# sedaprotocol/bn254

Hardware: AMD Instinct MI355X
Metric: BN254 pairings/sec (batch verify) (higher is better)
Workload: dtype u32

## Files before the change

### bn254_amd/csrc/bn254_hip.hip

```cpp
#include <hip/hip_runtime.h>
#include <thread>

#include <cstdio>
#include <cstdlib>
#include <cstring>
#include <new>

#include "../../include/bn254_hip.h"
#include "bn254_hash.h"
#include "bn254_io.h"
#include "bn254_pairing.h"

using namespace bn254;

#include "bn254_ws.h"
#include "bn254_lane.h"
#include "bn254_host.h"

KERNEL_SMALL void k_decode_g1(const uint8_t* pts, size_t n, uint32_t flags, Ws ws, int px, int inf_plane, int accumulate) {
  size_t i = (size_t)blockIdx.x * BN_WAVE + threadIdx.x;
  if (i >= n) return;
  G1Affine p;
  uint8_t st = decode_g1(p, pts + 64 * i, flags);
  if (st != ST_OK) g1_set_generator(p);
  ws_store_g1(ws, px, inf_plane, i, p);
  uint8_t prev = accumulate ? ws_byte(ws, BY_ST_DECODE, i) : (uint8_t)ST_OK;
  ws_byte(ws, BY_ST_DECODE, i) = prev != ST_OK ? prev : st;
}
KERNEL void k_decode_g2(const uint8_t* pts, size_t n, uint32_t flags, Ws ws, int accumulate) {
  size_t i = (size_t)blockIdx.x * BN_WAVE + threadIdx.x;
// ... 11 lines not shown
}

__device__ __forceinline__ bool msg_span(const uint64_t* off, size_t i, uint64_t msgs_len, uint64_t& lo, uint64_t& len) {
  lo = off[i];
  const uint64_t hi = off[i + 1];
  const bool ok = lo <= hi && hi <= msgs_len;
  len = ok ? hi - lo : 0;
  if (!ok) lo = 0;
  return ok;
}
KERNEL_SMALL void k_hash_init(size_t n, Ws ws) {
  size_t i = (size_t)blockIdx.x * BN_WAVE + threadIdx.x;
  if (i < n) { ws.h_best[i] = HASH_NONE; ws.h_next[i] = 0; }
  if (i <= HASH_MAX_ROUNDS) ws.h_cnt[i] = (i == 0) ? (uint32_t)n : 0u;
}
KERNEL_SMALL void k_hash_round(const uint8_t* msgs, const uint64_t* off, uint64_t msgs_len, Ws ws, int round, uint32_t width, uint32_t max_ctr) {
  const uint32_t n_act = ws.h_cnt[round];
  if (n_act == 0) return;
  const uint32_t* list = round == 0 ? nullptr : ws.h_list + (size_t)(round & 1) * ws.stride;
  const size_t total = (size_t)n_act * width;
  for (size_t w = (size_t)blockIdx.x * BN_WAVE + threadIdx.x; w < total; w += (size_t)gridDim.x * BN_WAVE) {
    uint32_t slot = (uint32_t)(w % n_act), j = (uint32_t)(w / n_act);
    uint32_t i = list ? list[slot] : slot;
    uint32_t ctr = (uint32_t)ws.h_next[i] + j;
    if (ctr >= max_ctr) continue;
    uint64_t lo, len;
    msg_span(off, i, msgs_len, lo, len);
    const uint8_t* msg = msgs + lo;
    HashState hs;
    hash_state_init(hs, msg, len);
    if (hash_try_filter(hs, msg, len, ctr)) atomicMin(&ws.h_best[i], ctr);
  }
}
KERNEL_SMALL void k_hash_resolve(Ws ws, int round, uint32_t width, uint32_t max_ctr, uint32_t mark) {
  const uint32_t n_act = ws.h_cnt[round];
  if (n_act == 0) return;
  const uint32_t* list = round == 0 ? nullptr : ws.h_list + (size_t)(round & 1) * ws.stride;
  uint32_t* list_out = ws.h_list + (size_t)((round + 1) & 1) * ws.stride;
  const size_t span = (size_t)gridDim.x * BN_WAVE;
  for (size_t base = (size_t)blockIdx.x * BN_WAVE; base < n_act; base += span) {
    const size_t slot = base + threadIdx.x;
    bool survivor = false;
    uint32_t i = 0;
    if (slot < n_act) {
      i = list ? list[slot] : (uint32_t)slot;
      if (ws.h_best[i] == HASH_NONE) {
        const uint32_t next = (uint32_t)ws.h_next[i] + width;
// ... 111 lines not shown
  ws_byte(ws, BY_ST_HASH, i) = ok ? (uint8_t)ST_OK : !span_ok ? (uint8_t)ST_INVALID_LENGTH : (uint8_t)ST_HASH_TO_POINT;
  if (tries_out) tries_out[i] = ok ? (uint8_t)(best + 1) : !span_ok ? (uint8_t)0 : (uint8_t)max_ctr;
}
KERNEL_SMALL void k_hash_finish(const uint8_t* msgs, const uint64_t* off, uint64_t msgs_len, size_t n, Ws ws, uint32_t max_ctr, int px, int inf_plane,
                                uint8_t* tries_out) {
  size_t i = (size_t)blockIdx.x * BN_WAVE + threadIdx.x;
  if (i >= n) return;
  hash_finish_item(msgs, off, msgs_len, i, ws, max_ctr, px, inf_plane, tries_out);
}
__device__ __noinline__ bool hash_try_msg(G1Affine& out, const uint8_t* msg, uint64_t len, uint32_t ctr) {
  HashState hs;
  hash_state_init(hs, msg, len);
  return hash_try(out, hs, msg, len, ctr);
}
KERNEL_SMALL void k_hash_finish_tail(const uint8_t* msgs, const uint64_t* off, uint64_t msgs_len, size_t n, Ws ws, uint32_t max_ctr, int px, int inf_plane,
                                     uint8_t* tries_out, unsigned nblk_finish, uint32_t chunk) {
  if (blockIdx.x < nblk_finish) {
    const size_t i = (size_t)blockIdx.x * BN_WAVE + threadIdx.x;
    if (i < n) hash_finish_item(msgs, off, msgs_len, i, ws, max_ctr, px, inf_plane, tries_out);
    return;
  }
  const uint32_t n_tail = ws.h_cnt[1];
  const uint32_t* list = ws.h_list + ws.stride;
  const uint32_t per_wave = BN_WAVE / chunk, sub = threadIdx.x / chunk, j = threadIdx.x % chunk;
  const size_t span = (size_t)(gridDim.x - nblk_finish) * per_wave;
  for (size_t base = (size_t)(blockIdx.x - nblk_finish) * per_wave; base < n_tail; base += span) {
    const size_t slot = base + sub;
    const bool live = slot < n_tail;
    uint32_t i = 0, first = 0;
    uint64_t lo = 0, len = 0;
    bool span_ok = true;
    if (live) { i = list[slot]; first = ws.h_next[i]; span_ok = msg_span(off, i, msgs_len, lo, len); }
    const uint8_t* msg = msgs + lo;
    bool open = live && span_ok;
    for (uint32_t k = 0;; k += chunk) {
      const uint32_t ctr = first + k + j;
      bool ok = false;
      G1Affine p;
// ... 323 lines not shown
  return 0;
}

int launch_decode_g2(bn254_ctx* c, hipStream_t s, const uint8_t* d_pts, size_t n, uint32_t flags, int accumulate) {
  if (c->pair_lanes && (flags & FLAG_G2_SUBGROUP_CHECK)) {
    if (route_lane_machine_helpers(c, n)) {
      k_decode_g2<<<grid_for(n), BN_WAVE, 0, s>>>(d_pts, n, flags & ~(uint32_t)FLAG_G2_SUBGROUP_CHECK, c->ws, accumulate);
      return bn254_lm_g2_subgroup(n, c->ws, s);
    }
    return bn254_pair_decode_g2(d_pts, n, flags, c->ws, accumulate, s);
  }
  k_decode_g2<<<grid_for(n), BN_WAVE, 0, s>>>(d_pts, n, flags, c->ws, accumulate);
  return 0;
}

static uint32_t hash_wide_width(size_t n) {
  double survivors = (double)n * 0.5274 * 0.5274 * 0.5274 * 0.5274;
  uint32_t w = 4;
  for (; w < 8 && (double)n / BN_WAVE + survivors * HASH_TAIL_CHUNK_DEFAULT / BN_WAVE > (double)HASH_WIDE_WAVES; ++w) survivors *= 0.5274;
  return w;
}
int launch_hash_rounds(bn254_ctx* c, hipStream_t s, const uint8_t* d_msgs, const uint64_t* d_off, size_t n, int px, int inf_plane,
                              uint8_t* d_tries, int mark_finish) {
  const uint32_t max_ctr = c->hash_max_tries ? (uint32_t)c->hash_max_tries : 255u;
  const uint64_t msgs_len = c->msgs_len_call;
  k_hash_init<<<grid_for(n > HASH_MAX_ROUNDS + 1 ? n : HASH_MAX_ROUNDS + 1), BN_WAVE, 0, s>>>(n, c->ws);
  if (n <= HASH_DIRECT_MAX_N && c->hash_direct_width > 0) {
    const uint32_t width = (uint32_t)c->hash_direct_width;
    k_hash_direct<<<grid_for(n * width), BN_WAVE, 0, s>>>(d_msgs, d_off, msgs_len, n, c->ws, width, max_ctr, px, inf_plane, d_tries);
    if (max_ctr > width)
      k_hash_round<<<grid_for(64 * (max_ctr - width)), BN_WAVE, 0, s>>>(d_msgs, d_off, msgs_len, c->ws, 1, max_ctr - width, max_ctr);
    if (mark_finish >= 0 && c->profiling) HIP_TRY(hipEventRecord(c->ev[mark_finish], s));
    k_hash_finish<<<grid_for(n), BN_WAVE, 0, s>>>(d_msgs, d_off, msgs_len, n, c->ws, max_ctr, px, inf_plane, d_tries);
    HIP_TRY(hipGetLastError());
    return 0;
  }
  if (n > HASH_DIRECT_MAX_N && (c->hash_schedule == 2 || (c->hash_schedule == 0 && n <= HASH_WIDE_MAX_N))) {
    uint32_t w0 = c->hash_wide_width ? (uint32_t)c->hash_wide_width : hash_wide_width(n);
    if (w0 > max_ctr) w0 = max_ctr;
    size_t lanes = n * w0;
    if (lanes > HASH_MAX_GRID_LANES) lanes = HASH_MAX_GRID_LANES;
    k_hash_round<<<grid_for(lanes), BN_WAVE, 0, s>>>(d_msgs, d_off, msgs_len, c->ws, 0, w0, max_ctr);
    if (n > HASH_RESOLVE_TILES_MIN) {
      size_t tiles = (n + HASH_RESOLVE_WG - 1) / HASH_RESOLVE_WG;
      if (tiles > 16384) tiles = 16384;
      k_hash_resolve_tiles<<<(unsigned)tiles, HASH_RESOLVE_WG, 0, s>>>(c->ws, 0, w0, max_ctr, HASH_TAIL);
    } else {
      k_hash_resolve<<<grid_for(n), BN_WAVE, 0, s>>>(c->ws, 0, w0, max_ctr, HASH_TAIL);
    }
    double pf = 1.0;
    for (uint32_t t = 0; t < w0 && pf > 1e-12; ++t) pf *= 0.5274;
    double bound = (double)n * pf * 1.25 + 256.0;
    if (bound > (double)n) bound = (double)n;
    const uint32_t chunk = (uint32_t)c->hash_tail_chunk;
    size_t tail_blocks = ((size_t)bound * chunk + BN_WAVE - 1) / BN_WAVE;
    if (tail_blocks > HASH_TAIL_MAX_BLOCKS) tail_blocks = HASH_TAIL_MAX_BLOCKS;
    if (mark_finish >= 0 && c->profiling) HIP_TRY(hipEventRecord(c->ev[mark_finish], s));
    const unsigned nblk = grid_for(n);
    k_hash_finish_tail<<<nblk + (unsigned)tail_blocks, BN_WAVE, 0, s>>>(d_msgs, d_off, msgs_len, n, c->ws, max_ctr, px, inf_plane, d_tries, nblk, chunk);
    HIP_TRY(hipGetLastError());
    return 0;
  }
  double expect = (double)n;
  uint32_t consumed = 0;
  for (int round = 0; round < HASH_MAX_ROUNDS && consumed < max_ctr; ++round) {
    bool last = round == HASH_MAX_ROUNDS - 1;
    double lanes_per_msg = (double)HASH_TARGET_LANES / (expect < 1.0 ? 1.0 : expect);
    uint32_t width = lanes_per_msg < 2.0 ? 1u : (uint32_t)lanes_per_msg;
    if (width > max_ctr - consumed || last) width = max_ctr - consumed;
    double bound = expect * 1.25 + 256.0;
    if (bound > (double)n) bound = (double)n;
    size_t lanes = (size_t)(bound * width);
    if (lanes > HASH_MAX_GRID_LANES) lanes = HASH_MAX_GRID_LANES;
    k_hash_round<<<grid_for(lanes), BN_WAVE, 0, s>>>(d_msgs, d_off, msgs_len, c->ws, round, width, max_ctr);
    if ((size_t)bound > HASH_RESOLVE_TILES_MIN) {
      size_t tiles = ((size_t)bound + HASH_RESOLVE_WG - 1) / HASH_RESOLVE_WG;
      if (tiles > 16384) tiles = 16384;
      k_hash_resolve_tiles<<<(unsigned)tiles, HASH_RESOLVE_WG, 0, s>>>(c->ws, round, width, max_ctr, HASH_NONE);
    } else {
      k_hash_resolve<<<grid_for((size_t)bound), BN_WAVE, 0, s>>>(c->ws, round, width, max_ctr, HASH_NONE);
    }
    consumed += width;
    double pf = 1.0;
    for (uint32_t t = 0; t < width && pf > 1e-12; ++t) pf *= 0.5274;
    expect *= pf;
  }
  if (mark_finish >= 0 && c->profiling) HIP_TRY(hipEventRecord(c->ev[mark_finish], s));
  k_hash_finish<<<grid_for(n), BN_WAVE, 0, s>>>(d_msgs, d_off, msgs_len, n, c->ws, max_ctr, px, inf_plane, d_tries);
  HIP_TRY(hipGetLastError());
  return 0;
}

int launch_decode_g1(bn254_ctx* c, hipStream_t s, const uint8_t* d_pts, size_t n, uint32_t flags, int px, int inf_plane, int accumulate) {
  k_decode_g1<<<grid_for(n), BN_WAVE, 0, s>>>(d_pts, n, flags, c->ws, px, inf_plane, accumulate);
  return 0;
}
int launch_miller_var_lane(bn254_ctx* c, hipStream_t s, size_t n) {
  k_miller_var<<<grid_for(n), BN_WAVE, 0, s>>>(n, c->ws);
  return 0;
}
int launch_miller_verify_lane(bn254_ctx* c, hipStream_t s, size_t n, const uint32_t* map, const uint32_t* count) {
// ... 29 lines not shown
  c->agg_rand_min_pairs = AGG_RAND_MIN_PAIRS_DEFAULT;
  c->agg_rand_group_pairs = AGG_RAND_GROUP_PAIRS_DEFAULT;
  c->bmr_min_tuples = BITMAP_RAND_MIN_TUPLES_DEFAULT;
  c->bmr_group_tuples = BITMAP_RAND_GROUP_TUPLES_DEFAULT;
  c->bmr_max_keys = BITMAP_RAND_MAX_KEYS_DEFAULT;
  c->collect_wave_min = COLLECT_WAVE_MIN_SHARES_DEFAULT;
  c->collect_rand_min_shares = COLLECT_RAND_MIN_SHARES_DEFAULT;
  c->collect_rand_min_per_key = COLLECT_RAND_MIN_PER_KEY_DEFAULT;
  c->collect_opt_min_shares = COLLECT_OPT_MIN_SHARES_DEFAULT;
  c->collect_opt_min_tuple_shares = COLLECT_OPT_MIN_TUPLE_SHARES_DEFAULT;
  c->merge_wave_min = MERGE_WAVE_MIN_PARTS_DEFAULT;
  c->merge_opt_min_parts = MERGE_OPT_MIN_PARTS_DEFAULT;
  c->trio_max_batch = TRIO_MAX_BATCH_DEFAULT;
  c->hash_direct_width = HASH_DIRECT_WIDTH_DEFAULT;
  c->hash_tail_chunk = HASH_TAIL_CHUNK_DEFAULT;
  c->trio_wave_roles = TRIO_WAVE_ROLES_DEFAULT;
  c->agg_subset_min_tuples = AGG_SUBSET_MIN_TUPLES_DEFAULT;
  c->agg_sort_by_msg = 1;
  c->agg_t4_route = 0;
  c->agg_wide_min_tuples = AGG_WIDE_MIN_TUPLES_DEFAULT;
  c->pinned_staging = PINNED_STAGING_DEFAULT;
  c->fits_w8 = bn254_quad_fits_device(1); c->fits_quad = bn254_quad_fits_device(0); c->fits_trio = bn254_trio_fits_device();
  if (c->trio_wave_roles == 2 && !c->fits_w8) c->trio_wave_roles = 1;
  if (c->trio_wave_roles == 1 && !c->fits_quad) c->trio_wave_roles = 0;
  if (!c->fits_trio) c->trio_max_batch = 0;
  c->nonet_max_batch = bn254_nonet_fits_device() ? NONET_MAX_BATCH_DEFAULT : 0;
  c->lm_max_batch = bn254_lm_fits_device() ? LM_MAX_BATCH_DEFAULT : 0;
  c->nonet_wide = 1;
  c->g2_fixed_base = 1;
  c->key_dedup = 1;
// ... 105 lines not shown
  if (option == BN254_OPT_TRIO_MAX_BATCH) {
    if (value < 0 || (value > 0 && !c->fits_trio)) return BN254_E_BAD_ARGUMENT;
    c->trio_max_batch = value;
    return 0;
  }
  if (option == BN254_OPT_TRIO_WAVE_ROLES) {
    if (value < 0 || value > 2 || (value == 2 && !c->fits_w8) || (value == 1 && !c->fits_quad)) return BN254_E_BAD_ARGUMENT;
    c->trio_wave_roles = value;
    return 0;
  }
  if (option == BN254_OPT_HASH_DIRECT_WIDTH) {
    if (value < 0 || value > 32 || (value & (value - 1))) return BN254_E_BAD_ARGUMENT;
    c->hash_direct_width = value;
    return 0;
  }
  if (option == BN254_OPT_HASH_SCHEDULE) { if (value < 0 || value > 2) return BN254_E_BAD_ARGUMENT; c->hash_schedule = value; return 0; }
  if (option == BN254_OPT_HASH_WIDE_WIDTH) { if (value < 0 || value > 64) return BN254_E_BAD_ARGUMENT; c->hash_wide_width = value; return 0; }
  if (option == BN254_OPT_HASH_TAIL_CHUNK) {
    if (value < 2 || value > 32 || (value & (value - 1))) return BN254_E_BAD_ARGUMENT;
    c->hash_tail_chunk = value;
    return 0;
  }
  if (option == BN254_OPT_NONET_MAX_BATCH) {
    HIP_TRY(hipSetDevice(c->device));
    if (value < 0 || (value > 0 && !bn254_nonet_fits_device())) return BN254_E_BAD_ARGUMENT;
    c->nonet_max_batch = value;
    return 0;
  }
  if (option == BN254_OPT_NONET_WIDE) { c->nonet_wide = value != 0; return 0; }
  if (option == BN254_OPT_LM_MAX_BATCH) {
    HIP_TRY(hipSetDevice(c->device));
    if (value < 0 || (value > 0 && !bn254_lm_fits_device())) return BN254_E_BAD_ARGUMENT;
// ... 128 lines not shown
    PROF_MARK(3);
    if ((rc = bn254_pair_final_exp(n, c->ws, 1, d_status, nullptr, nullptr, s))) return rc;
    HIP_TRY(hipEventRecord(c->kd_done, s));
  } else if (split) {
    const unsigned g = grid_for(n);
    k_miller_verify_split<<<2 * g, BN_WAVE, 0, s>>>(n, c->ws.stride / 2, g, c->ws);
    PROF_MARK(3);
    k_final_exp<<<g, BN_WAVE, 0, s>>>(n, 2, 1, c->ws.stride / 2, c->ws, 1, nullptr, d_status, 0, 0, nullptr, nullptr);
  } else if ((rc = launch_verify_miller_fe(c, s, n, BN_PAIRS_VERIFY, 1, d_status, true))) return rc;
  PROF_MARK(4);
  prof_done(c, hash_first ? EV_HASH_FIRST : EV_DECODE_FIRST);
  HIP_TRY(hipGetLastError());
  return 0;
}
static int verify_after_decode(bn254_ctx* c, hipStream_t s, const uint8_t* d_msgs, const uint64_t* d_off, size_t n, uint8_t* d_status, bool split,
                               const KeyDedup* kd = nullptr) {
  PROF_MARK(1);
  if (const int rc = launch_hash_rounds(c, s, d_msgs, d_off, n, PL_P2X, BY_P2_INF, nullptr)) return rc;
  PROF_MARK(2);
  return verify_tail(c, s, n, d_status, split, kd, 0);
}

int bn254_batch_verify_device(bn254_ctx* c, const uint8_t* d_msgs, const uint64_t* d_off, const uint8_t* d_sigs, const uint8_t* d_pks,
                              size_t n, uint32_t flags, uint8_t* d_status, void* stream) {
  MsgsLenScope msgs_len_scope(c);
  if (!c || (n && (!d_msgs || !d_off || !d_sigs || !d_pks || !d_status))) return BN254_E_BAD_ARGUMENT;
  if (n == 0) return 0;
  if (misaligned(d_sigs) || misaligned(d_pks) || ((uintptr_t)d_off & 7u)) return BN254_E_MISALIGNED;
  HIP_TRY(hipSetDevice(c->device));
  bool split = c->split_miller && n <= BN_SPLIT_MAX_N;
  bool key_dedup = c->key_dedup && c->kd_max_keys > 0 && c->pair_lanes && !split && n <= 0xFFFFFFFFu &&
                         route_for(c, n).miller == BN_ML_LANE_PAIRS && route_for(c, n).fe == BN_FE_LANE_PAIRS;
  if (const size_t chunk = ws_chunk_for(c, n, split ? 2 : 1, key_dedup))
// ... 7 lines not shown
    rc = kd_reserve(c, n, kd);
    if (rc == KD_NO_ROOM) key_dedup = false;
    else if (rc) return rc;
    rc = 0;
  }
  c->kd_last_run = key_dedup;
  hipStream_t s = stream ? (hipStream_t)stream : c->stream;
  CallDone call_done(c, s);
  PROF_MARK(0);
  if (key_dedup) {
    HIP_TRY(hipStreamWaitEvent(s, c->kd_done, 0));
    const bool cache_reset = !c->kd_cache || !c->kd_cache_valid || c->kd_cache_flags != flags || c->kd_cache_max_keys != c->kd_max_keys ||
                             c->kd_cache_hash_bits != c->kd_hash_bits;
    c->kd_cache_valid = false;
    HIP_TRY(hipEventRecord(c->kd_fork, s));
    HIP_TRY(hipStreamWaitEvent(c->kd_stream, c->kd_fork, 0));
    if ((rc = bn254_kd_enqueue(d_pks, n, flags, kd, c->kd_force_generic, cache_reset, c->kd_cache, c->kd_stream))) return rc;
    HIP_TRY(hipEventRecord(c->kd_join, c->kd_stream));
    c->kd_cache_valid = c->kd_cache != 0;
    c->kd_cache_flags = flags; c->kd_cache_max_keys = c->kd_max_keys; c->kd_cache_hash_bits = c->kd_hash_bits;
  }
  k_decode_g1<<<grid_for(n), BN_WAVE, 0, s>>>(d_sigs, n, flags, c->ws, PL_P1X, BY_P1_INF, 0);
  if ((rc = launch_decode_g2(c, s, d_pks, n, flags, 1))) return rc;
  return verify_after_decode(c, s, d_msgs, d_off, n, d_status, split, key_dedup ? &kd : nullptr);
}

int bn254_batch_verify_compressed_device(bn254_ctx* c, const uint8_t* d_msgs, const uint64_t* d_off, const uint8_t* d_sigs33,
                                         const uint8_t* d_pks65, size_t n, uint8_t* d_status, void* stream) {
  MsgsLenScope msgs_len_scope(c);
  if (!c || (n && (!d_msgs || !d_off || !d_sigs33 || !d_pks65 || !d_status))) return BN254_E_BAD_ARGUMENT;
  if (n == 0) return 0;
  if ((uintptr_t)d_off & 7u) return BN254_E_MISALIGNED;
  HIP_TRY(hipSetDevice(c->device));
  if (const size_t chunk = ws_chunk_for(c, n))
    return verify_device_sliced(n, chunk, [&](size_t lo, size_t len) {
// ... 266 lines not shown
```

### bn254_amd/csrc/bn254_host.h

```cpp
#pragma once
#include <hip/hip_runtime.h>

#include <cstdint>
#include <cstdlib>
#include <cstring>
#include <new>

#include "../../include/bn254_hip.h"

#define BN_HIDDEN __attribute__((visibility("hidden")))

struct AggTables { int valid; size_t n_msgs, n_signers, n_groups, groups4, built_for; int wide2, wide1, t4_builder; };

struct AggrLast { size_t ng, cbase, tbase; const uint32_t *nagg, *bkey; const uint64_t *glo, *ghi; const uint8_t* gst; };

enum EvLayout { EV_DECODE_FIRST = 0, EV_HASH_FIRST = 1, EV_COLLECT = 2 };

struct bn254_ctx {
  int device;
  hipStream_t stream;
  Ws ws;
  uint8_t* stage[8];
  size_t stage_cap[8];
  int profiling;
  int split_miller;
  Pool pool[8];
  size_t pool_fp[8];
  int agg_wide_min_tuples;
  int agg_subset_min_tuples;
  int agg_sort_by_msg;
  int agg_t4_route;
  int pair_lanes;
  int rand_min_batch;
  int rand_items_per_lane;
  int hash_max_tries;
  int trio_wave_roles;
  int hash_direct_width;
  int hash_schedule;
  int hash_wide_width;
  int hash_tail_chunk;
  int trio_max_batch;
  int lm_max_batch;
  int nonet_wide;
  int nonet_max_batch;
  hipEvent_t ev[5];
  int ev_valid;
  int ev_layout;
  hipStream_t copy_stream;
  uint8_t* pin;
  size_t pin_cap;
  int pinned_staging;
  hipEvent_t copy_done;
  uint64_t msgs_len_next;
  int msgs_len_declared;
// ... 158 lines not shown
  HostStaging(const HostStaging&) = delete;
  HostStaging& operator=(const HostStaging&) = delete;
 private:
  hipError_t drain();
  struct Back { void* host; const void* dev; size_t bytes; } back[6];
  int n_back = 0;
  bool finished = false;
};


static inline void prof_done(bn254_ctx* c, int layout) { if (c->profiling) { c->ev_valid = 1; c->ev_layout = layout; } }
#define PROF_MARK(idx) do { if (c->profiling) HIP_TRY(hipEventRecord(c->ev[idx], s)); } while (0)

BN_HIDDEN int launch_decode_g1(bn254_ctx* c, hipStream_t s, const uint8_t* d_pts, size_t n, uint32_t flags, int px, int inf_plane, int accumulate);
BN_HIDDEN int launch_decode_g2(bn254_ctx* c, hipStream_t s, const uint8_t* d_pts, size_t n, uint32_t flags, int accumulate);
BN_HIDDEN int launch_hash_rounds(bn254_ctx* c, hipStream_t s, const uint8_t* d_msgs, const uint64_t* d_off, size_t n, int px, int inf_plane,
                                 uint8_t* d_tries, int mark_finish = -1);
BN_HIDDEN int launch_final_exp_layout(bn254_ctx* c, hipStream_t s, size_t n, int use_hash, uint8_t* d_status, int fe);
enum BnVerifyPairs { BN_PAIRS_VERIFY = 0, BN_PAIRS_CHECK_PKS = 1 };
BN_HIDDEN int launch_verify_miller_fe(bn254_ctx* c, hipStream_t s, size_t n, int pairs, int use_hash, uint8_t* d_status, bool mark);
BN_HIDDEN int launch_keyed_miller_fe(bn254_ctx* c, hipStream_t s, size_t n, const uint32_t* d_key_idx, uint8_t* d_status);
BN_HIDDEN int launch_keyed_no_keys(bn254_ctx* c, hipStream_t s, size_t n, uint8_t* d_status);
struct RandSeed { uint32_t w[8]; };
static inline RandSeed rand_seed_from(const uint8_t* seed32) {
  RandSeed seed;
  for (int j = 0; j < 8; ++j)
    seed.w[j] = ((uint32_t)seed32[4 * j] << 24) | ((uint32_t)seed32[4 * j + 1] << 16) | ((uint32_t)seed32[4 * j + 2] << 8) | seed32[4 * j + 3];
  return seed;
}
static inline int rand_mode_of(uint32_t flags) { return (flags & BN254_FLAG_RAND64) ? 1 : (flags & BN254_FLAG_RAND_GLV) ? 2 : 0; }
struct KeyedRandNeed { size_t gbase, groups_max, ws_entries, words; };
static inline KeyedRandNeed keyed_rand_need(const bn254_ctx* c, size_t n) {
// ... 39 lines not shown
```

### bn254_amd/csrc/bn254_ws.h

```cpp
#pragma once
#include <stddef.h>

#define BN_WAVE 64
#define BN_SPLIT_MAX_N ((size_t)98304)
#define TRIO_MAX_BATCH_DEFAULT 16384
#define NONET_WIDE_MAX_BATCH 1024
#define NONET_MAX_BATCH_DEFAULT 3072
#define LM_MAX_BATCH_DEFAULT 1536
enum BnMillerLayout { BN_ML_LANE_MACHINE = 0, BN_ML_WAVE_ROLES = 1, BN_ML_LANE_PAIRS = 2 };
enum BnFeLayout { BN_FE_NONET_WIDE = 0, BN_FE_NONET = 1, BN_FE_OCTET = 2, BN_FE_LANE_PAIRS = 3 };
struct BnRouteLimits { size_t lm_max, nonet_wide_max, nonet_max, small_max; };
struct BnRoute { int miller, fe; };
static inline BnRoute bn_route(const BnRouteLimits& L, size_t n) {
  BnRoute r = {BN_ML_LANE_PAIRS, BN_FE_LANE_PAIRS};
  if (n > L.small_max) return r;
  r.miller = n <= L.lm_max ? BN_ML_LANE_MACHINE : BN_ML_WAVE_ROLES;
  r.fe = n <= L.nonet_max ? (n <= L.nonet_wide_max ? BN_FE_NONET_WIDE : BN_FE_NONET) : BN_FE_OCTET;
  return r;
}
static inline int bn_route_table(const BnRouteLimits& L, size_t* max_n, BnRoute* route, int cap) {
  size_t b[4] = {L.lm_max, L.nonet_wide_max, L.nonet_max, L.small_max};
  for (int i = 0; i < 4; ++i) if (b[i] > L.small_max) b[i] = L.small_max;
  for (int i = 0; i < 4; ++i) for (int j = i + 1; j < 4; ++j) if (b[j] < b[i]) { size_t t = b[i]; b[i] = b[j]; b[j] = t; }
  int rows = 0;
// ... 47 lines not shown
  do {                                                                                           \
    if ((ws).clk && threadIdx.x == 0 && blockIdx.x < BN_CLK_MAX_WG) {                            \
      unsigned long long* p_ = (ws).clk + ((size_t)(slot) * BN_CLK_MAX_WG + blockIdx.x) * 2;    \
      p_[0] += clock64() - clk0_; p_[1] += wall_clock64() - wall0_;                              \
    }                                                                                            \
  } while (0)
#define HASH_NONE 0xFFFFFFFFu
#define HASH_DONE 0xFFFFFFFEu
#define HASH_TAIL 0xFFFFFFFDu
#define HASH_DIRECT_WIDTH_DEFAULT 32
#define HASH_DIRECT_MAX_N ((size_t)4096)
#define HASH_MAX_ROUNDS 64
#define HASH_MAX_GRID_LANES ((size_t)1 << 24)
#ifndef HASH_TARGET_LANES
#define HASH_TARGET_LANES ((size_t)1 << 17)
#endif
#ifndef HASH_WIDE_MAX_N
#define HASH_WIDE_MAX_N ((size_t)32768)
#endif
#define HASH_WIDE_WAVES 1024
#define HASH_TAIL_CHUNK_DEFAULT 32
#define HASH_TAIL_MAX_BLOCKS ((size_t)16384)
enum { PL_P1X = 0, PL_P1Y, PL_QX0, PL_QX1, PL_QY0, PL_QY1, PL_P2X, PL_P2Y, PL_HASHX, PL_HASHY, PL_F0, N_PLANES = PL_F0 + 12 };
enum { BY_ST_DECODE = 0, BY_ST_HASH, BY_P1_INF, BY_Q_INF, BY_P2_INF, BY_A_INF, N_BYTE_PLANES };

__device__ __forceinline__ Fp ws_load_fp(const Ws& ws, int plane, size_t i) {
  Fp r;
#pragma unroll
  for (int k = 0; k < BN_LIMBS; ++k) r.v[k] = ws.planes[((size_t)plane * BN_LIMBS + k) * ws.stride + i];
  return r;
// ... 173 lines not shown
```

### bn254_amd/engine.py

```python
import ctypes

from . import _native

G1_BYTES, G2_BYTES, GT_BYTES, SCALAR_BYTES = 64, 128, 384, 32
FLAG_G2_SUBGROUP_CHECK = 1
FLAG_REJECT_IDENTITY = 2
FLAG_RAND64 = 0x100
FLAG_RAND_GLV = 0x200
OPT_SPLIT_MILLER = 1
OPT_HASH_MAX_TRIES = 2
OPT_RAND_ITEMS_PER_LANE = 3
OPT_PAIR_LANES = 4
OPT_RAND_MIN_BATCH = 5
OPT_TRIO_MAX_BATCH = 6
OPT_HASH_DIRECT_WIDTH = 7
OPT_TRIO_WAVE_ROLES = 8
OPT_AGG_SUBSET_MIN_TUPLES = 9
OPT_CLOCK_PROBE = 10
OPT_AGG_SORT_BY_MSG = 11
OPT_PINNED_STAGING = 12
OPT_NONET_MAX_BATCH = 13
OPT_LM_MAX_BATCH = 15
OPT_NONET_WIDE = 16
OPT_AGG_WIDE_MIN_TUPLES = 14
OPT_MAX_CHUNK = 17
OPT_ASSUME_FREE_MB = 18
OPT_G2_FIXED_BASE = 19
OPT_KEY_DEDUP = 20
OPT_KEY_DEDUP_MAX_KEYS = 21
OPT_KEY_DEDUP_MIN_MULT = 22
OPT_KEY_DEDUP_FORCE_GENERIC = 23
OPT_KEY_DEDUP_HASH_BITS = 24
OPT_AGGD_KEYED_ROUTE = 25
OPT_AGG_RAND_MIN_PAIRS = 26
OPT_AGG_RAND_GROUP_PAIRS = 27
OPT_BITMAP_TABLE_MAX_KEYS = 28
OPT_BITMAP_ROUTE = 29
OPT_HASH_SCHEDULE = 30
OPT_HASH_WIDE_WIDTH = 31
OPT_HASH_TAIL_CHUNK = 32
OPT_BITMAP_RAND_MIN_TUPLES = 33
OPT_BITMAP_RAND_GROUP_TUPLES = 34
OPT_BITMAP_RAND_MAX_KEYS = 35
OPT_KEY_DEDUP_FOLD = 44
OPT_KEY_CACHE = 36
OPT_COLLECT_RAND_MIN_SHARES = 38
OPT_COLLECT_RAND_MIN_PER_KEY = 39
COLLECT_RAND_MIN_SHARES_DEFAULT = 65664
COLLECT_RAND_MIN_PER_KEY_DEFAULT = 42
OPT_COLLECT_OPT_MIN_SHARES = 40
OPT_AGG_T4_ROUTE = 42
OPT_COLLECT_OPT_MIN_TUPLE_SHARES = 41
COLLECT_OPT_MIN_SHARES_DEFAULT = 1539
COLLECT_OPT_MIN_TUPLE_SHARES_DEFAULT = 1
# ... 807 lines not shown
```

### include/bn254_hip.h

```cpp
#ifndef BN254_HIP_H
#define BN254_HIP_H

#include <stddef.h>
#include <stdint.h>

#ifdef __cplusplus
extern "C" {
#endif

typedef struct bn254_ctx bn254_ctx;

#define BN254_FLAG_G2_SUBGROUP_CHECK 1u
#define BN254_FLAG_REJECT_IDENTITY 2u
#define BN254_FLAG_RAND64 0x100u
#define BN254_FLAG_RAND_GLV 0x200u

#define BN254_E_BAD_ARGUMENT (-10001)
#define BN254_E_MISALIGNED (-10002)
#define BN254_E_NO_DEVICE (-10003)
#define BN254_E_RCCL (-10004)
#define BN254_E_NO_MEMORY (-10005)

#define BN254_OK 0
#define BN254_ERR_HASH_TO_POINT 1
// ... 250 lines not shown
                             uint32_t flags, uint8_t *gt , uint8_t *status , uint64_t *checksum );
int bn254_mgpu_batch_pairing_device(bn254_mgpu *mg, const uint8_t *const *d_g1, const uint8_t *const *d_g2, size_t n, size_t k,
                                    uint32_t flags, uint8_t *const *d_gt, uint8_t *const *d_status_all, uint64_t *const *d_checksum,
                                    void *const *streams);
int bn254_mgpu_batch_hash_to_g1(bn254_mgpu *mg, const uint8_t *msgs, const uint64_t *msg_off, size_t n, uint8_t *points ,
                                uint8_t *status , uint8_t *tries );

#ifndef BN254_NO_DEV_HOOKS
#define BN254_OPT_SPLIT_MILLER 1
#define BN254_OPT_PAIR_LANES 4
#define BN254_OPT_RAND_ITEMS_PER_LANE 3
#define BN254_OPT_TRIO_WAVE_ROLES 8
#define BN254_OPT_HASH_DIRECT_WIDTH 7
#define BN254_OPT_HASH_SCHEDULE 30
#define BN254_OPT_HASH_WIDE_WIDTH 31
#define BN254_OPT_HASH_TAIL_CHUNK 32
#define BN254_OPT_NONET_WIDE 16
#define BN254_OPT_AGG_SORT_BY_MSG 11
#define BN254_OPT_CLOCK_PROBE 10
#define BN254_OPT_HASH_MAX_TRIES 2
#define BN254_OPT_G2_FIXED_BASE 19
#define BN254_OPT_KEY_DEDUP_FORCE_GENERIC 23
#define BN254_OPT_KEY_DEDUP_FOLD 44
#define BN254_OPT_KEY_DEDUP_HASH_BITS 24
#define BN254_OPT_AGGD_KEYED_ROUTE 25
#define BN254_OPT_AGG_RAND_GROUP_PAIRS 27
#define BN254_OPT_BITMAP_RAND_GROUP_TUPLES 34
#define BN254_OPT_BITMAP_ROUTE 29
#define BN254_OPT_AGG_T4_ROUTE 42
#define BN254_OPT_ASSUME_FREE_MB 18
// ... 32 lines not shown
```

Baseline: 15.86 million.

## Add two-round hash schedule and launch hash front before key-dedup fork

Adds a two-round hash-to-G1 schedule for mid-sized batches. It sizes the first round from a target lane count and runs that round with a waves-per-EU-4 kernel variant, then runs a second round over the survivors before the tail finish. It also splits launch_hash_rounds into front and rest parts, so decode and the first hash round can be enqueued on the main stream before the key-dedup side stream is forked, letting them overlap with key dedup. The aim is fewer wasted hash lanes and less serialization, at the cost of extra kernel launches and a more complex schedule. Resolve-launch and plan math are factored into helpers.

```diff
diff --git a/bn254_amd/csrc/bn254_hash_plan.h b/bn254_amd/csrc/bn254_hash_plan.h
--- /dev/null
+++ b/bn254_amd/csrc/bn254_hash_plan.h
@@ -0,0 +1,56 @@
+#pragma once
+#include <cstddef>
+#include <cstdint>
+
+#define HASH_P_FAIL 0.5274
+#define HASH_TWO_ROUND_LANES0 ((size_t)1 << 18)
+#define HASH_TWO_ROUND_LANES1 ((size_t)1 << 17)
+#define HASH_TWO_ROUND_W1_MAX 24
+#define HASH_ROUND_WIDTH_MAX 64
+
+static inline double hash_p_fail_pow(uint32_t width) {
+  double pf = 1.0;
+  for (uint32_t t = 0; t < width && pf > 1e-12; ++t) pf *= HASH_P_FAIL;
+  return pf;
+}
+static inline size_t hash_survivor_bound(double expect, size_t n) {
+  const double bound = expect * 1.25 + 256.0;
+  return bound > (double)n ? n : (size_t)bound;
+}
+static inline size_t hash_tail_blocks(size_t bound, uint32_t chunk) {
+  const size_t blocks = (bound * chunk + BN_WAVE - 1) / BN_WAVE;
+  return blocks > HASH_TAIL_MAX_BLOCKS ? HASH_TAIL_MAX_BLOCKS : blocks;
+}
+static inline uint32_t hash_wide_width(size_t n) {
+  double survivors = (double)n * HASH_P_FAIL * HASH_P_FAIL * HASH_P_FAIL * HASH_P_FAIL;
+  uint32_t w = 4;
+  for (; w < 8 && (double)n / BN_WAVE + survivors * HASH_TAIL_CHUNK_DEFAULT / BN_WAVE > (double)HASH_WIDE_WAVES; ++w) survivors *= HASH_P_FAIL;
+  return w;
+}
+
+struct HashTwoRoundPlan {
+  uint32_t w0, w1;
+  size_t lanes0, lanes1;
+  size_t bound1, bound2;
+  size_t tail_blocks;
+};
+static inline HashTwoRoundPlan hash_two_round_plan(size_t n, uint32_t max_ctr, uint32_t w0_opt, uint32_t w1_opt, uint32_t chunk) {
+  HashTwoRoundPlan p;
+  size_t w0 = w0_opt ? w0_opt : HASH_TWO_ROUND_LANES0 / (n ? n : 1);
+  if (w0 > HASH_ROUND_WIDTH_MAX) w0 = HASH_ROUND_WIDTH_MAX;
+  if (w0 > max_ctr) w0 = max_ctr;
+  if (w0 < 1) w0 = 1;
+  p.w0 = (uint32_t)w0;
+  const double expect1 = (double)n * hash_p_fail_pow(p.w0);
+  size_t w1 = w1_opt ? w1_opt : (size_t)((double)HASH_TWO_ROUND_LANES1 / (expect1 < 1.0 ? 1.0 : expect1));
+  if (w1 > (w1_opt ? HASH_ROUND_WIDTH_MAX : HASH_TWO_ROUND_W1_MAX)) w1 = w1_opt ? HASH_ROUND_WIDTH_MAX : HASH_TWO_ROUND_W1_MAX;
+  if (w1 > (size_t)(max_ctr > p.w0 ? max_ctr - p.w0 : 0)) w1 = max_ctr > p.w0 ? max_ctr - p.w0 : 0;
+  if (w1 < 1) w1 = 1;
+  p.w1 = (uint32_t)w1;
+  p.lanes0 = n * p.w0 > HASH_MAX_GRID_LANES ? HASH_MAX_GRID_LANES : n * p.w0;
+  p.bound1 = hash_survivor_bound(expect1, n);
+  p.lanes1 = p.bound1 * p.w1 > HASH_MAX_GRID_LANES ? HASH_MAX_GRID_LANES : p.bound1 * p.w1;
+  p.bound2 = hash_survivor_bound(expect1 * hash_p_fail_pow(p.w1), n);
+  p.tail_blocks = hash_tail_blocks(p.bound2, chunk);
+  return p;
+}
diff --git a/bn254_amd/csrc/bn254_hip.hip b/bn254_amd/csrc/bn254_hip.hip
--- a/bn254_amd/csrc/bn254_hip.hip
+++ b/bn254_amd/csrc/bn254_hip.hip
@@ -14,6 +14,7 @@
 using namespace bn254;
 
 #include "bn254_ws.h"
+#include "bn254_hash_plan.h"
 #include "bn254_lane.h"
 #include "bn254_host.h"
 
@@ -55,7 +56,8 @@
   if (i < n) { ws.h_best[i] = HASH_NONE; ws.h_next[i] = 0; }
   if (i <= HASH_MAX_ROUNDS) ws.h_cnt[i] = (i == 0) ? (uint32_t)n : 0u;
 }
-KERNEL_SMALL void k_hash_round(const uint8_t* msgs, const uint64_t* off, uint64_t msgs_len, Ws ws, int round, uint32_t width, uint32_t max_ctr) {
+__device__ __forceinline__ void hash_round_body(const uint8_t* msgs, const uint64_t* off, uint64_t msgs_len, const Ws& ws, int round, uint32_t width,
+                                                uint32_t max_ctr) {
   const uint32_t n_act = ws.h_cnt[round];
   if (n_act == 0) return;
   const uint32_t* list = round == 0 ? nullptr : ws.h_list + (size_t)(round & 1) * ws.stride;
@@ -72,6 +74,13 @@
     hash_state_init(hs, msg, len);
     if (hash_try_filter(hs, msg, len, ctr)) atomicMin(&ws.h_best[i], ctr);
   }
+}
+KERNEL_SMALL void k_hash_round(const uint8_t* msgs, const uint64_t* off, uint64_t msgs_len, Ws ws, int round, uint32_t width, uint32_t max_ctr) {
+  hash_round_body(msgs, off, msgs_len, ws, round, width, max_ctr);
+}
+__global__ __launch_bounds__(BN_WAVE) __attribute__((amdgpu_waves_per_eu(4, 4)))
+void k_hash_round4(const uint8_t* msgs, const uint64_t* off, uint64_t msgs_len, Ws ws, int round, uint32_t width, uint32_t max_ctr) {
+  hash_round_body(msgs, off, msgs_len, ws, round, width, max_ctr);
 }
 KERNEL_SMALL void k_hash_resolve(Ws ws, int round, uint32_t width, uint32_t max_ctr, uint32_t mark) {
   const uint32_t n_act = ws.h_cnt[round];
@@ -213,14 +222,14 @@
   return hash_try(out, hs, msg, len, ctr);
 }
 KERNEL_SMALL void k_hash_finish_tail(const uint8_t* msgs, const uint64_t* off, uint64_t msgs_len, size_t n, Ws ws, uint32_t max_ctr, int px, int inf_plane,
-                                     uint8_t* tries_out, unsigned nblk_finish, uint32_t chunk) {
+                                     uint8_t* tries_out, unsigned nblk_finish, uint32_t chunk, int tail_round) {
   if (blockIdx.x < nblk_finish) {
     const size_t i = (size_t)blockIdx.x * BN_WAVE + threadIdx.x;
     if (i < n) hash_finish_item(msgs, off, msgs_len, i, ws, max_ctr, px, inf_plane, tries_out);
     return;
   }
-  const uint32_t n_tail = ws.h_cnt[1];
-  const uint32_t* list = ws.h_list + ws.stride;
+  const uint32_t n_tail = ws.h_cnt[tail_round];
+  const uint32_t* list = ws.h_list + (size_t)(tail_round & 1) * ws.stride;
   const uint32_t per_wave = BN_WAVE / chunk, sub = threadIdx.x / chunk, j = threadIdx.x % chunk;
   const size_t span = (size_t)(gridDim.x - nblk_finish) * per_wave;
   for (size_t base = (size_t)(blockIdx.x - nblk_finish) * per_wave; base < n_tail; base += span) {
@@ -574,20 +583,25 @@
   return 0;
 }
 
-static uint32_t hash_wide_width(size_t n) {
-  double survivors = (double)n * 0.5274 * 0.5274 * 0.5274 * 0.5274;
-  uint32_t w = 4;
-  for (; w < 8 && (double)n / BN_WAVE + survivors * HASH_TAIL_CHUNK_DEFAULT / BN_WAVE > (double)HASH_WIDE_WAVES; ++w) survivors *= 0.5274;
-  return w;
+static void launch_hash_resolve(bn254_ctx* c, hipStream_t s, int round, size_t bound, uint32_t width, uint32_t max_ctr, uint32_t mark) {
+  if (bound > HASH_RESOLVE_TILES_MIN) {
+    size_t tiles = (bound + HASH_RESOLVE_WG - 1) / HASH_RESOLVE_WG;
+    if (tiles > 16384) tiles = 16384;
+    k_hash_resolve_tiles<<<(unsigned)tiles, HASH_RESOLVE_WG, 0, s>>>(c->ws, round, width, max_ctr, mark);
+  } else {
+    k_hash_resolve<<<grid_for(bound), BN_WAVE, 0, s>>>(c->ws, round, width, max_ctr, mark);
+  }
 }
 int launch_hash_rounds(bn254_ctx* c, hipStream_t s, const uint8_t* d_msgs, const uint64_t* d_off, size_t n, int px, int inf_plane,
-                              uint8_t* d_tries, int mark_finish) {
+                              uint8_t* d_tries, int mark_finish, int part) {
   const uint32_t max_ctr = c->hash_max_tries ? (uint32_t)c->hash_max_tries : 255u;
   const uint64_t msgs_len = c->msgs_len_call;
-  k_hash_init<<<grid_for(n > HASH_MAX_ROUNDS + 1 ? n : HASH_MAX_ROUNDS + 1), BN_WAVE, 0, s>>>(n, c->ws);
+  const bool front = part != HASH_REST, rest = part != HASH_FRONT;
+  if (front) k_hash_init<<<grid_for(n > HASH_MAX_ROUNDS + 1 ? n : HASH_MAX_ROUNDS + 1), BN_WAVE, 0, s>>>(n, c->ws);
   if (n <= HASH_DIRECT_MAX_N && c->hash_direct_width > 0) {
     const uint32_t width = (uint32_t)c->hash_direct_width;
-    k_hash_direct<<<grid_for(n * width), BN_WAVE, 0, s>>>(d_msgs, d_off, msgs_len, n, c->ws, width, max_ctr, px, inf_plane, d_tries);
+    if (front) k_hash_direct<<<grid_for(n * width), BN_WAVE, 0, s>>>(d_msgs, d_off, msgs_len, n, c->ws, width, max_ctr, px, inf_plane, d_tries);
+    if (!rest) { HIP_TRY(hipGetLastError()); return 0; }
     if (max_ctr > width)
       k_hash_round<<<grid_for(64 * (max_ctr - width)), BN_WAVE, 0, s>>>(d_msgs, d_off, msgs_len, c->ws, 1, max_ctr - width, max_ctr);
     if (mark_finish >= 0 && c->profiling) HIP_TRY(hipEventRecord(c->ev[mark_finish], s));
@@ -600,24 +614,28 @@
     if (w0 > max_ctr) w0 = max_ctr;
     size_t lanes = n * w0;
     if (lanes > HASH_MAX_GRID_LANES) lanes = HASH_MAX_GRID_LANES;
-    k_hash_round<<<grid_for(lanes), BN_WAVE, 0, s>>>(d_msgs, d_off, msgs_len, c->ws, 0, w0, max_ctr);
-    if (n > HASH_RESOLVE_TILES_MIN) {
-      size_t tiles = (n + HASH_RESOLVE_WG - 1) / HASH_RESOLVE_WG;
-      if (tiles > 16384) tiles = 16384;
-      k_hash_resolve_tiles<<<(unsigned)tiles, HASH_RESOLVE_WG, 0, s>>>(c->ws, 0, w0, max_ctr, HASH_TAIL);
-    } else {
-      k_hash_resolve<<<grid_for(n), BN_WAVE, 0, s>>>(c->ws, 0, w0, max_ctr, HASH_TAIL);
-    }
-    double pf = 1.0;
-    for (uint32_t t = 0; t < w0 && pf > 1e-12; ++t) pf *= 0.5274;
-    double bound = (double)n * pf * 1.25 + 256.0;
-    if (bound > (double)n) bound = (double)n;
+    if (front) k_hash_round<<<grid_for(lanes), BN_WAVE, 0, s>>>(d_msgs, d_off, msgs_len, c->ws, 0, w0, max_ctr);
+    if (!rest) { HIP_TRY(hipGetLastError()); return 0; }
+    launch_hash_resolve(c, s, 0, n, w0, max_ctr, HASH_TAIL);
     const uint32_t chunk = (uint32_t)c->hash_tail_chunk;
-    size_t tail_blocks = ((size_t)bound * chunk + BN_WAVE - 1) / BN_WAVE;
-    if (tail_blocks > HASH_TAIL_MAX_BLOCKS) tail_blocks = HASH_TAIL_MAX_BLOCKS;
+    const size_t tail_blocks = hash_tail_blocks(hash_survivor_bound((double)n * hash_p_fail_pow(w0), n), chunk);
     if (mark_finish >= 0 && c->profiling) HIP_TRY(hipEventRecord(c->ev[mark_finish], s));
     const unsigned nblk = grid_for(n);
-    k_hash_finish_tail<<<nblk + (unsigned)tail_blocks, BN_WAVE, 0, s>>>(d_msgs, d_off, msgs_len, n, c->ws, max_ctr, px, inf_plane, d_tries, nblk, chunk);
+    k_hash_finish_tail<<<nblk + (unsigned)tail_blocks, BN_WAVE, 0, s>>>(d_msgs, d_off, msgs_len, n, c->ws, max_ctr, px, inf_plane, d_tries, nblk, chunk, 1);
+    HIP_TRY(hipGetLastError());
+    return 0;
+  }
+  if (n > HASH_DIRECT_MAX_N && (c->hash_schedule == 3 || (c->hash_schedule == 0 && n <= HASH_TWO_ROUND_MAX_N))) {
+    const uint32_t chunk = (uint32_t)c->hash_tail_chunk;
+    const HashTwoRoundPlan p = hash_two_round_plan(n, max_ctr, (uint32_t)c->hash_wide_width, (uint32_t)c->hash_round1_width, chunk);
+    if (front) k_hash_round4<<<grid_for(p.lanes0), BN_WAVE, 0, s>>>(d_msgs, d_off, msgs_len, c->ws, 0, p.w0, max_ctr);
+    if (!rest) { HIP_TRY(hipGetLastError()); return 0; }
+    launch_hash_resolve(c, s, 0, n, p.w0, max_ctr, HASH_NONE);
+    k_hash_round<<<grid_for(p.lanes1), BN_WAVE, 0, s>>>(d_msgs, d_off, msgs_len, c->ws, 1, p.w1, max_ctr);
+    launch_hash_resolve(c, s, 1, p.bound1, p.w1, max_ctr, HASH_TAIL);
+    if (mark_finish >= 0 && c->profiling) HIP_TRY(hipEventRecord(c->ev[mark_finish], s));
+    const unsigned nblk = grid_for(n);
+    k_hash_finish_tail<<<nblk + (unsigned)p.tail_blocks, BN_WAVE, 0, s>>>(d_msgs, d_off, msgs_len, n, c->ws, max_ctr, px, inf_plane, d_tries, nblk, chunk, 2);
     HIP_TRY(hipGetLastError());
     return 0;
   }
@@ -632,19 +650,13 @@
     if (bound > (double)n) bound = (double)n;
     size_t lanes = (size_t)(bound * width);
     if (lanes > HASH_MAX_GRID_LANES) lanes = HASH_MAX_GRID_LANES;
-    k_hash_round<<<grid_for(lanes), BN_WAVE, 0, s>>>(d_msgs, d_off, msgs_len, c->ws, round, width, max_ctr);
-    if ((size_t)bound > HASH_RESOLVE_TILES_MIN) {
-      size_t tiles = ((size_t)bound + HASH_RESOLVE_WG - 1) / HASH_RESOLVE_WG;
-      if (tiles > 16384) tiles = 16384;
-      k_hash_resolve_tiles<<<(unsigned)tiles, HASH_RESOLVE_WG, 0, s>>>(c->ws, round, width, max_ctr, HASH_NONE);
-    } else {
-      k_hash_resolve<<<grid_for((size_t)bound), BN_WAVE, 0, s>>>(c->ws, round, width, max_ctr, HASH_NONE);
-    }
+    if (round == 0 ? front : rest) k_hash_round<<<grid_for(lanes), BN_WAVE, 0, s>>>(d_msgs, d_off, msgs_len, c->ws, round, width, max_ctr);
+    if (!rest) { HIP_TRY(hipGetLastError()); return 0; }
+    launch_hash_resolve(c, s, round, (size_t)bound, width, max_ctr, HASH_NONE);
     consumed += width;
-    double pf = 1.0;
-    for (uint32_t t = 0; t < width && pf > 1e-12; ++t) pf *= 0.5274;
-    expect *= pf;
-  }
+    expect *= hash_p_fail_pow(width);
+  }
+  if (!rest) { HIP_TRY(hipGetLastError()); return 0; }
   if (mark_finish >= 0 && c->profiling) HIP_TRY(hipEventRecord(c->ev[mark_finish], s));
   k_hash_finish<<<grid_for(n), BN_WAVE, 0, s>>>(d_msgs, d_off, msgs_len, n, c->ws, max_ctr, px, inf_plane, d_tries);
   HIP_TRY(hipGetLastError());
@@ -704,6 +716,7 @@
   c->trio_max_batch = TRIO_MAX_BATCH_DEFAULT;
   c->hash_direct_width = HASH_DIRECT_WIDTH_DEFAULT;
   c->hash_tail_chunk = HASH_TAIL_CHUNK_DEFAULT;
+  c->hash_front_first = VERIFY_HASH_FRONT_FIRST_DEFAULT;
   c->trio_wave_roles = TRIO_WAVE_ROLES_DEFAULT;
   c->agg_subset_min_tuples = AGG_SUBSET_MIN_TUPLES_DEFAULT;
   c->agg_sort_by_msg = 1;
@@ -839,8 +852,10 @@
     c->hash_direct_width = value;
     return 0;
   }
-  if (option == BN254_OPT_HASH_SCHEDULE) { if (value < 0 || value > 2) return BN254_E_BAD_ARGUMENT; c->hash_schedule = value; return 0; }
-  if (option == BN254_OPT_HASH_WIDE_WIDTH) { if (value < 0 || value > 64) return BN254_E_BAD_ARGUMENT; c->hash_wide_width = value; return 0; }
+  if (option == BN254_OPT_HASH_SCHEDULE) { if (value < 0 || value > 3) return BN254_E_BAD_ARGUMENT; c->hash_schedule = value; return 0; }
+  if (option == BN254_OPT_HASH_WIDE_WIDTH) { if (value < 0 || value > HASH_ROUND_WIDTH_MAX) return BN254_E_BAD_ARGUMENT; c->hash_wide_width = value; return 0; }
+  if (option == BN254_OPT_HASH_ROUND1_WIDTH) { if (value < 0 || value > HASH_ROUND_WIDTH_MAX) return BN254_E_BAD_ARGUMENT; c->hash_round1_width = value; return 0; }
+  if (option == BN254_OPT_VERIFY_HASH_FRONT_FIRST) { if (value < 0 || value > 1) return BN254_E_BAD_ARGUMENT; c->hash_front_first = value; return 0; }
   if (option == BN254_OPT_HASH_TAIL_CHUNK) {
     if (value < 2 || value > 32 || (value & (value - 1))) return BN254_E_BAD_ARGUMENT;
     c->hash_tail_chunk = value;
@@ -999,9 +1014,9 @@
   return 0;
 }
 static int verify_after_decode(bn254_ctx* c, hipStream_t s, const uint8_t* d_msgs, const uint64_t* d_off, size_t n, uint8_t* d_status, bool split,
-                               const KeyDedup* kd = nullptr) {
-  PROF_MARK(1);
-  if (const int rc = launch_hash_rounds(c, s, d_msgs, d_off, n, PL_P2X, BY_P2_INF, nullptr)) return rc;
+                               const KeyDedup* kd = nullptr, bool front_done = false) {
+  if (!front_done) PROF_MARK(1);
+  if (const int rc = launch_hash_rounds(c, s, d_msgs, d_off, n, PL_P2X, BY_P2_INF, nullptr, -1, front_done ? HASH_REST : HASH_ALL)) return rc;
   PROF_MARK(2);
   return verify_tail(c, s, n, d_status, split, kd, 0);
 }
@@ -1039,11 +1054,19 @@
                              c->kd_cache_hash_bits != c->kd_hash_bits;
     c->kd_cache_valid = false;
     HIP_TRY(hipEventRecord(c->kd_fork, s));
+    const bool front_first = c->hash_front_first != 0;
+    if (front_first) {
+      k_decode_g1<<<grid_for(n), BN_WAVE, 0, s>>>(d_sigs, n, flags, c->ws, PL_P1X, BY_P1_INF, 0);
+      if ((rc = launch_decode_g2(c, s, d_pks, n, flags, 1))) return rc;
+      PROF_MARK(1);
+      if ((rc = launch_hash_rounds(c, s, d_msgs, d_off, n, PL_P2X, BY_P2_INF, nullptr, -1, HASH_FRONT))) return rc;
+    }
     HIP_TRY(hipStreamWaitEvent(c->kd_stream, c->kd_fork, 0));
     if ((rc = bn254_kd_enqueue(d_pks, n, flags, kd, c->kd_force_generic, cache_reset, c->kd_cache, c->kd_stream))) return rc;
     HIP_TRY(hipEventRecord(c->kd_join, c->kd_stream));
     c->kd_cache_valid = c->kd_cache != 0;
     c->kd_cache_flags = flags; c->kd_cache_max_keys = c->kd_max_keys; c->kd_cache_hash_bits = c->kd_hash_bits;
+    if (front_first) return verify_after_decode(c, s, d_msgs, d_off, n, d_status, split, &kd, true);
   }
   k_decode_g1<<<grid_for(n), BN_WAVE, 0, s>>>(d_sigs, n, flags, c->ws, PL_P1X, BY_P1_INF, 0);
   if ((rc = launch_decode_g2(c, s, d_pks, n, flags, 1))) return rc;
diff --git a/bn254_amd/csrc/bn254_host.h b/bn254_amd/csrc/bn254_host.h
--- a/bn254_amd/csrc/bn254_host.h
+++ b/bn254_amd/csrc/bn254_host.h
@@ -38,6 +38,8 @@
   int hash_direct_width;
   int hash_schedule;
   int hash_wide_width;
+  int hash_round1_width;
+  int hash_front_first;
   int hash_tail_chunk;
   int trio_max_batch;
   int lm_max_batch;
@@ -226,8 +228,9 @@
 
 BN_HIDDEN int launch_decode_g1(bn254_ctx* c, hipStream_t s, const uint8_t* d_pts, size_t n, uint32_t flags, int px, int inf_plane, int accumulate);
 BN_HIDDEN int launch_decode_g2(bn254_ctx* c, hipStream_t s, const uint8_t* d_pts, size_t n, uint32_t flags, int accumulate);
+enum HashPart { HASH_ALL = 0, HASH_FRONT = 1, HASH_REST = 2 };
 BN_HIDDEN int launch_hash_rounds(bn254_ctx* c, hipStream_t s, const uint8_t* d_msgs, const uint64_t* d_off, size_t n, int px, int inf_plane,
-                                 uint8_t* d_tries, int mark_finish = -1);
+                                 uint8_t* d_tries, int mark_finish = -1, int part = HASH_ALL);
 BN_HIDDEN int launch_final_exp_layout(bn254_ctx* c, hipStream_t s, size_t n, int use_hash, uint8_t* d_status, int fe);
 enum BnVerifyPairs { BN_PAIRS_VERIFY = 0, BN_PAIRS_CHECK_PKS = 1 };
 BN_HIDDEN int launch_verify_miller_fe(bn254_ctx* c, hipStream_t s, size_t n, int pairs, int use_hash, uint8_t* d_status, bool mark);
diff --git a/bn254_amd/csrc/bn254_ws.h b/bn254_amd/csrc/bn254_ws.h
--- a/bn254_amd/csrc/bn254_ws.h
+++ b/bn254_amd/csrc/bn254_ws.h
@@ -85,6 +85,12 @@
 #define HASH_MAX_GRID_LANES ((size_t)1 << 24)
 #ifndef HASH_TARGET_LANES
 #define HASH_TARGET_LANES ((size_t)1 << 17)
+#endif
+#ifndef VERIFY_HASH_FRONT_FIRST_DEFAULT
+#define VERIFY_HASH_FRONT_FIRST_DEFAULT 1
+#endif
+#ifndef HASH_TWO_ROUND_MAX_N
+#define HASH_TWO_ROUND_MAX_N ((size_t)32768)
 #endif
 #ifndef HASH_WIDE_MAX_N
 #define HASH_WIDE_MAX_N ((size_t)32768)
diff --git a/bn254_amd/engine.py b/bn254_amd/engine.py
--- a/bn254_amd/engine.py
+++ b/bn254_amd/engine.py
@@ -38,6 +38,8 @@
 OPT_BITMAP_ROUTE = 29
 OPT_HASH_SCHEDULE = 30
 OPT_HASH_WIDE_WIDTH = 31
+OPT_HASH_ROUND1_WIDTH = 46
+OPT_VERIFY_HASH_FRONT_FIRST = 47
 OPT_HASH_TAIL_CHUNK = 32
 OPT_BITMAP_RAND_MIN_TUPLES = 33
 OPT_BITMAP_RAND_GROUP_TUPLES = 34
diff --git a/include/bn254_hip.h b/include/bn254_hip.h
--- a/include/bn254_hip.h
+++ b/include/bn254_hip.h
@@ -288,6 +288,8 @@
 #define BN254_OPT_HASH_DIRECT_WIDTH 7
 #define BN254_OPT_HASH_SCHEDULE 30
 #define BN254_OPT_HASH_WIDE_WIDTH 31
+#define BN254_OPT_HASH_ROUND1_WIDTH 46
+#define BN254_OPT_VERIFY_HASH_FRONT_FIRST 47
 #define BN254_OPT_HASH_TAIL_CHUNK 32
 #define BN254_OPT_NONET_WIDE 16
 #define BN254_OPT_AGG_SORT_BY_MSG 11
```

New measurement: 15.94 million (median of 6 runs). No clear change (+0.5%).
